# anonymousauthors001/SGS-GNN

Hardware: AMD Instinct MI355X
Metric: sampled edges/sec + training steps/sec, Reddit hybrid 20% sparsity (higher is better)
Workload: dtype f32

## Files before the change

include/sgs_hip.h:

```cpp
#ifndef SGS_HIP_H_
#define SGS_HIP_H_

#include <stddef.h>
#include <stdint.h>

#ifdef __cplusplus
extern "C" {
#endif

#define SGS_ABI_VERSION 1

#define SGS_OK 0
#define SGS_EINVAL (-1)
#define SGS_EWORKSPACE (-2)
#define SGS_EHIP (-3)

typedef void* sgs_stream_t;

int sgs_abi_version(void);
const char* sgs_last_error(void);

int sgs_rng_set_epoch_buffer(const uint64_t* epoch_dev);
int sgs_exp_noise(uint64_t seed, uint64_t stream_id, int64_t E, float* noise, sgs_stream_t stream);
int sgs_dropout_keep(uint64_t seed, uint32_t site, int64_t rows, int64_t cols, float p, uint8_t* keep,
// ... 74 lines not shown

int sgs_mean_weights(int64_t n_edges, int64_t N, const int32_t* in_ptr, const int32_t* out_ptr, const int32_t* out_dst,
                     float* what_in, float* what_out, sgs_stream_t stream);
int sgs_degree_prior_logits(const int64_t* edge_index, int64_t E, int64_t N, const int32_t* in_ptr,
                            const int32_t* out_ptr, float* logits, sgs_stream_t stream);

size_t sgs_gcn_norm_bwd_workspace_bytes(int64_t N);
int sgs_gcn_norm_bwd(const float* w, const float* gw_hat, const float* gloop, int64_t n_edges, int64_t N,
                     const float* dis, const float* loopw, const int32_t* in_ptr, const int32_t* in_src,
                     const int32_t* in_eid, const int32_t* out_ptr, const int32_t* out_dst, const int32_t* out_eid,
                     const int32_t* loop_eid, const int64_t* edge_index, float* dw, void* ws, size_t ws_bytes,
                     sgs_stream_t stream);
int sgs_gcn_norm_bwd_sum(const float* w, const float* gw_hat, const float* gloop, const float* gw_hat2, const float* gloop2, const float* dw_add,
                         int64_t n_edges, int64_t N, const float* dis, const float* loopw, const int32_t* in_ptr, const int32_t* in_src,
                         const int32_t* in_eid, const int32_t* out_ptr, const int32_t* out_dst, const int32_t* out_eid,
                         const int32_t* loop_eid, const int64_t* edge_index, float* dw, void* ws, size_t ws_bytes, sgs_stream_t stream);

int sgs_gcn_norm_bwd_node(const float* w, const float* gw_hat, const float* gloop, int64_t n_edges, int64_t N,
                          const float* dis, const float* loopw, const int32_t* in_ptr, const int32_t* in_src,
                          const int32_t* in_eid, const int32_t* out_ptr, const int32_t* out_dst, const int32_t* out_eid,
                          float* Hn, sgs_stream_t stream);
int sgs_gcn_norm_bwd_edge(const float* gw_hat, const float* gloop, int64_t n_edges, int64_t N, const float* dis,
                          const int32_t* loop_eid, const int64_t* edge_index, const float* Hn, float* dw,
                          sgs_stream_t stream);

#define SGS_ACT_NONE 0
#define SGS_ACT_RELU 1
#define SGS_ACT_RELU_DROPOUT 2
int sgs_spmm_csr(const float* X, int64_t N, int64_t D, int64_t nnz, const int32_t* ptr, const int32_t* col, const float* val,
                 const float* diag, const float* bias, int act, float p_drop, uint64_t seed, uint32_t site, float* Y,
                 sgs_stream_t stream);

int sgs_sddmm_csr(const float* A, const float* B, int64_t N, int64_t D, int64_t nnz, const int32_t* ptr, const int32_t* col,
                  const int32_t* eid, float* g, float* gdiag, sgs_stream_t stream);

int sgs_spmm_csr_variant(int64_t N, int64_t D, int64_t nnz, int aligned16);
int sgs_sddmm_csr_variant(int64_t N, int64_t D, int64_t nnz, int aligned16);

int sgs_act_bwd(const float* dY, const float* Y, int64_t n, int act, float p_drop, float* dZ, sgs_stream_t stream);
size_t sgs_colsum_workspace_bytes(int64_t N, int64_t D);
int sgs_colsum(const float* A, int64_t N, int64_t D, float* out, void* ws, size_t ws_bytes, sgs_stream_t stream);
int sgs_act_bwd_colsum(const float* dY, const float* Y, int64_t N, int64_t D, int act, float p_drop, float* dZ, float* colsum, void* ws,
                       size_t ws_bytes, sgs_stream_t stream);

int sgs_colsum_variant(int64_t N, int64_t D, int fused_act);

int sgs_gcn_pair_ok(int64_t N, int64_t nnz, int64_t D);
int sgs_spmm_csr_next(const float* X, int64_t N, int64_t D, int64_t nnz, const int32_t* ptr, const int32_t* col, const float* val,
                      const float* diag, const float* bias, int act, float p_drop, uint64_t seed, uint32_t site, const float* Wn, int64_t Dn,
                      float* Y, float* Z, sgs_stream_t stream);
int sgs_spmm_csr_bwd_prev(const float* dZ, int64_t N, int64_t D, int64_t nnz, const int32_t* ptr, const int32_t* col, const float* val,
                          const float* diag, const float* W, int64_t Dp, const float* Yp, int act, float p_drop, float* dX, float* dZp,
                          float* colsum, sgs_stream_t stream);

size_t sgs_edge_score_workspace_bytes(int64_t N, int64_t H, int64_t E);
int sgs_edge_score_hidden_supported(int64_t H);
int sgs_edge_score_get_variant(void);
int sgs_edge_score_get_bwd_variant(void);
void sgs_edge_score_set_bwd_variant(int variant);
int sgs_edge_score_bwd_tile(void);
void sgs_edge_score_set_variant(int variant);
int sgs_edge_score_fwd(const float* codes, const float* U, int64_t N, int64_t H, const int64_t* edge_index, int64_t E,
                       int64_t edge_id_offset, const float* W1, const float* b1, const float* w2, const float* b2,
                       float p_drop, uint64_t seed, uint32_t site, float* p_out, void* ws, size_t ws_bytes,
                       sgs_stream_t stream);
size_t sgs_edge_mates_workspace_bytes(int64_t n_edges);
int sgs_edge_mates(const int64_t* edge_index, int64_t n_edges, int64_t N, const int32_t* out_ptr, const int32_t* out_dst,
                   const int32_t* out_eid, int32_t* mate, void* ws, size_t ws_bytes, sgs_stream_t stream);
int sgs_edge_score_paired_supported(int64_t H);
int sgs_edge_score_fwd_paired(const float* codes, const float* U, int64_t N, int64_t H, const int64_t* edge_index, int64_t E,
                              int64_t edge_id_offset, const int32_t* canon, int64_t M, const int32_t* mate, const float* W1, const float* b1,
                              const float* w2, const float* b2, float p_drop, uint64_t seed, uint32_t site, float* p_out, void* ws,
                              size_t ws_bytes, sgs_stream_t stream);
int sgs_edge_score_bwd_core(const float* codes, const float* U, int64_t N, int64_t H, const int64_t* edge_index,
                            int64_t E, int64_t edge_id_offset, const int64_t* active_eid, int64_t n_active, const float* grad_p,
                            const float* W1, const float* b1, const float* w2, const float* b2, float p_drop,
                            uint64_t seed, uint32_t site, float* dv, float* hdz_part, float* dz, float* feat, void* ws,
                            size_t ws_bytes, sgs_stream_t stream);
int sgs_edge_score_bwd_dfeat_supported(int64_t H);
int sgs_edge_score_bwd_dfeat(const float* dv, int64_t n, int64_t H, const float* W1, float* dfeat, void* ws, size_t ws_bytes,
                             sgs_stream_t stream);

int sgs_edge_score_bwd_bits_supported(int64_t H);
int sgs_edge_score_fwd_mask(const float* codes, const float* U, int64_t N, int64_t H, const int64_t* edge_index, int64_t E,
                            int64_t edge_id_offset, const int32_t* canon, int64_t M, const int32_t* mate, const float* W1, const float* b1,
                            const float* w2, const float* b2, float p_drop, uint64_t seed, uint32_t site, float* p_out, uint32_t* maskbits,
                            void* ws, size_t ws_bytes, sgs_stream_t stream);
int sgs_edge_score_bwd_prep(const float* codes, int64_t N, int64_t H, const int64_t* edge_index, int64_t E, const int64_t* active_eid,
                            int64_t n_active, const float* grad_p, const float* p, const uint32_t* maskbits, float* dz, uint32_t* dvbits,
                            float* feat, sgs_stream_t stream);
int sgs_edge_score_dw2_from_parts(const float* W1, const float* T_raw, const float* U, const float* R_raw, const float* b1, const float* c_raw,
                                  int64_t N, int64_t H, float p_drop, float* dw2, sgs_stream_t stream);
int sgs_edge_score_probe_set(int stagger, int prio, uint32_t mode_mask);
int sgs_edge_score_probe_trace(unsigned long long* buf);
size_t sgs_edge_score_epd_workspace_bytes(int64_t H);
int sgs_edge_score_epd_fwd(const float* A, int64_t N, int64_t H, const int64_t* edge_index, int64_t E, int64_t edge_id_offset, const float* W1,
                           const float* b1, const float* w2, const float* b2, float p_hidden, uint64_t seed, uint32_t site, float p_ep,
                           uint64_t seed_x, uint32_t site_x, uint64_t seed_y, uint32_t site_y, float* p_out, void* ws, size_t ws_bytes,
                           sgs_stream_t stream);
int sgs_edge_score_epd_bwd_core(const float* A, int64_t N, int64_t H, const int64_t* edge_index, int64_t E, int64_t edge_id_offset,
                                const int64_t* active_eid, int64_t n_active, const float* grad_p, const float* W1, const float* b1, const float* w2,
                                const float* b2, float p_hidden, uint64_t seed, uint32_t site, float p_ep, uint64_t seed_x, uint32_t site_x,
                                uint64_t seed_y, uint32_t site_y, float* dv, float* hdz_part, float* dz, float* feat2, void* ws, size_t ws_bytes,
                                sgs_stream_t stream);
int sgs_edge_score_epd_reduce(const float* dfeat2, const float* A, int64_t N, int64_t H, const int32_t* in_ptr, const int32_t* in_src,
                              const int32_t* in_eid, const int32_t* out_ptr, const int32_t* out_dst, const int32_t* out_eid,
// ... 261 lines not shown
```

sgs-gnn_amd/csrc/gcn.hip:

```cpp
#include "sgs_common.h"

namespace sgs {
size_t graph_sort_workspace_bytes(int64_t n, int64_t N);
size_t graph_src_sorted_workspace_bytes(int64_t n, int64_t N);
int graph_build_src_sorted(const int64_t* ei, int64_t n, int64_t N, int32_t* in_ptr, int32_t* in_src, int32_t* in_eid, int32_t* out_ptr,
                           int32_t* out_dst, int32_t* out_eid, int32_t* loop_eid, int32_t* unsorted_flag, void* ws, size_t ws_bytes,
                           hipStream_t stream);
int graph_build_by_sort(const int64_t* ei, int64_t n, int64_t N, int32_t* in_ptr, int32_t* in_src, int32_t* in_eid, int32_t* out_ptr,
                        int32_t* out_dst, int32_t* out_eid, int32_t* loop_eid, void* ws, size_t ws_bytes, hipStream_t stream);
}

namespace sgs {
namespace {

constexpr int kT = 256;
constexpr int kMaxLdsRow = 8192;

__global__ void __launch_bounds__(kT) count_degrees(const int64_t* __restrict__ ei, int64_t n_edges, int* __restrict__ cnt_in,
                                                   int* __restrict__ cnt_out, int* __restrict__ loop_eid) {
    const int64_t e = static_cast<int64_t>(blockIdx.x) * kT + threadIdx.x;
    if (e >= n_edges) return;
    const int s = static_cast<int>(ei[e]), d = static_cast<int>(ei[n_edges + e]);
    atomicAdd(&cnt_in[d], 1);
    atomicAdd(&cnt_out[s], 1);
// ... 948 lines not shown
    norm_deg_body(w ? w + d * q : nullptr, N, in_ptr + d * (N + 1), in_src + d * q, in_eid + d * q, loop_eid + d * N, dis + d * N, loopw + d * N);
}
__global__ void __launch_bounds__(kT) multi_norm_weights(const float* __restrict__ w, int64_t q, int64_t N, const int* __restrict__ in_ptr,
                                                        const int* __restrict__ in_src, const int* __restrict__ in_eid, const float* __restrict__ dis,
                                                        const float* __restrict__ loopw, float* __restrict__ what_in, float* __restrict__ what_loop) {
    const int64_t d = blockIdx.y;
    norm_weights_body(N, w ? w + d * q : nullptr, N, q, in_ptr + d * (N + 1), in_src + d * q, in_eid + d * q, nullptr, nullptr, nullptr, dis + d * N,
                      loopw + d * N, what_in + d * q, nullptr, what_loop + d * N);
}
template <int VEC, int LPR>
__global__ void __launch_bounds__(kT) multi_spmm_csr(const float* __restrict__ X, int64_t xs, int64_t N, int64_t D, int64_t nnz,
                                                    const int* __restrict__ ptr, const int* __restrict__ col, const float* __restrict__ val,
                                                    const float* __restrict__ diag, const float* __restrict__ bias, int act, float* __restrict__ Y) {
    const int64_t d = blockIdx.y;
    spmm_csr_body<VEC, LPR>(X + d * xs, N, D, ptr + d * (N + 1), col + d * nnz, val + d * nnz, diag ? diag + d * N : nullptr, bias, act, 1.0f, 0u,
                            uint64_t(0), 0u, nullptr, Y + d * N * D);
}
template <int VEC, int NW>
__global__ void __launch_bounds__(64 * NW) multi_spmm_csr_rowblock(const float* __restrict__ X, int64_t xs, int64_t N, int64_t D, int64_t nnz,
                                                                 const int* __restrict__ ptr, const int* __restrict__ col,
                                                                 const float* __restrict__ val, const float* __restrict__ diag,
                                                                 const float* __restrict__ bias, int act, float* __restrict__ Y) {
    const int64_t d = blockIdx.y;
    spmm_csr_rowblock_body<VEC, NW>(X + d * xs, N, D, ptr + d * (N + 1), col + d * nnz, val + d * nnz, diag ? diag + d * N : nullptr, bias, act,
                                    1.0f, 0u, uint64_t(0), 0u, nullptr, Y + d * N * D);
}

enum { kPairCol = 0, kPairFwd = 1, kPairBwd = 2 };
constexpr int kPairMaxD = 512;
constexpr int kPairWlds = 12288;
constexpr int kPairWpre = kPairWlds / 1024;
template <class FY, class FW>
__device__ __forceinline__ float lib_gemm_dot(int K, FY y, FW w) {
    const int Kmain = K / 16 * 16;
    float z = 0.f;
    if (Kmain > 0) {
        float ya[8], wa[8];
#pragma unroll
        for (int u = 0; u < 8; ++u) { const int k = 2 * (u & 3) + (u >> 2); ya[u] = y(k); wa[u] = w(k); }
        for (int b = 0; b < Kmain; b += 8) {
            const int nb = b + 8 < Kmain ? b + 8 : b;
            float yn[8], wn[8];
#pragma unroll
            for (int u = 0; u < 8; ++u) { const int k = nb + 2 * (u & 3) + (u >> 2); yn[u] = y(k); wn[u] = w(k); }
#pragma unroll
            for (int u = 0; u < 8; ++u) z = fmaf(ya[u], wa[u], z);
#pragma unroll
            for (int u = 0; u < 8; ++u) { ya[u] = yn[u]; wa[u] = wn[u]; }
        }
    }
    for (int k = Kmain; k < K; ++k) z = fmaf(y(k), w(k), z);
    return z;
}
template <int VEC, int NW, int MODE>
__global__ void __launch_bounds__(1024) spmm_rowgroup_pair(const float* __restrict__ X, int64_t N, int64_t D, const int* __restrict__ ptr,
                                                           const int* __restrict__ col, const float* __restrict__ val,
                                                           const float* __restrict__ diag, const float* __restrict__ bias, int act,
                                                           float drop_scale, uint32_t drop_thresh, uint64_t seed, uint32_t site,
                                                           const uint64_t* __restrict__ epoch, float* __restrict__ Y,
                                                           const float* __restrict__ Wn, int64_t Dn, const float* __restrict__ Yp,
                                                           float* __restrict__ Zn, int ncs, float* __restrict__ colsum) {
    using V = typename VecT<VEC>::type;
    constexpr int RG = 16 / NW;
    __shared__ float part[RG][NW][64 * VEC];
    __shared__ __align__(16) float ys[RG * kPairMaxD];
    __shared__ float wl[MODE == kPairFwd ? kPairWlds : 1];
    if (MODE != kPairFwd && static_cast<int>(blockIdx.x) < ncs) {
        if (D % 4 == 0) colsum_small_v4_body<false>(X, nullptr, N, D, SGS_ACT_NONE, 1.f, nullptr, colsum, blockIdx.x);
        else            colsum_small_body<false>(X, nullptr, N, D, SGS_ACT_NONE, 1.f, nullptr, colsum, blockIdx.x);
        return;
    }
    seed = fold_epoch(seed, epoch);
    const int lane = threadIdx.x & 63, wave = (threadIdx.x >> 6) % NW, grp = threadIdx.x / (64 * NW);
    const int64_t row0 = static_cast<int64_t>(blockIdx.x - ncs) * RG;
    const int64_t i = row0 + grp;
    const bool live = i < N;
    int b = 0, e = 0;
    float dg = 0.f;
    uint32_t rkey = 0;
    const int yact = MODE == kPairBwd ? SGS_ACT_NONE : act;
    if (live) {
        b = ptr[i];
        e = ptr[i + 1];
        dg = diag ? diag[i] : 0.f;
        rkey = dropout_row_key(seed, site, static_cast<uint64_t>(i));
    }
    const bool wlds = MODE == kPairFwd && Dn * D <= kPairWlds;
    float wpre[MODE == kPairFwd ? kPairWpre : 1];
    if (MODE == kPairFwd && wlds) {
#pragma unroll
        for (int u = 0; u < kPairWpre; ++u) {
            const int64_t idx = threadIdx.x + 1024 * u;
            wpre[u] = idx < Dn * D ? Wn[idx] : 0.f;
        }
    }
    for (int64_t cbase = 0; cbase < D; cbase += 64 * VEC) {
        const int64_t c0 = cbase + static_cast<int64_t>(lane) * VEC;
        const bool in = c0 < D;
        float acc[VEC];
#pragma unroll
        for (int v = 0; v < VEC; ++v) acc[v] = 0.f;
        if (in) {
            int k = b + wave;
            for (; k + 7 * NW < e; k += 8 * NW) {
                int j[8]; float w[8]; V x[8];
#pragma unroll
                for (int u = 0; u < 8; ++u) { j[u] = col[k + NW * u]; w[u] = val[k + NW * u]; }
#pragma unroll
                for (int u = 0; u < 8; ++u) x[u] = *reinterpret_cast<const V*>(X + static_cast<int64_t>(j[u]) * D + c0);
#pragma unroll
                for (int u = 0; u < 8; ++u) {
                    float xv[VEC];
                    *reinterpret_cast<V*>(xv) = x[u];
#pragma unroll
                    for (int v = 0; v < VEC; ++v) acc[v] = fmaf(w[u], xv[v], acc[v]);
                }
            }
            for (; k < e; k += NW) {
                float xv[VEC];
                *reinterpret_cast<V*>(xv) = *reinterpret_cast<const V*>(X + static_cast<int64_t>(col[k]) * D + c0);
                const float w = val[k];
#pragma unroll
                for (int v = 0; v < VEC; ++v) acc[v] = fmaf(w, xv[v], acc[v]);
            }
        }
#pragma unroll
        for (int v = 0; v < VEC; ++v) part[grp][wave][lane * VEC + v] = acc[v];
        __syncthreads();
        const int t = threadIdx.x % (64 * NW);
        if (live && t < 64 * VEC && cbase + t < D) {
            const int64_t c = cbase + t;
            float y = 0.f;
#pragma unroll
            for (int g = 0; g < NW; g += 4) y += (part[grp][g][t] + part[grp][g + 1][t]) + (part[grp][g + 2][t] + part[grp][g + 3][t]);
            if (diag) y = fmaf(dg, X[i * D + c], y);
            if (bias) y += bias[c];
            if (yact != SGS_ACT_NONE) y = fmaxf(y, 0.f);
            if (yact == SGS_ACT_RELU_DROPOUT) y = dropout_keep_col(rkey, static_cast<uint32_t>(c), drop_thresh) ? y * drop_scale : 0.f;
            Y[i * D + c] = y;
            ys[grp * D + c] = y;
        }
        __syncthreads();
    }
    if (MODE == kPairFwd) {
        if (wlds) {
#pragma unroll
            for (int u = 0; u < kPairWpre; ++u) {
                const int64_t idx = threadIdx.x + 1024 * u;
                if (idx < Dn * D) {
                    const int64_t o = idx / D, k = idx - o * D;
                    wl[k * Dn + o] = wpre[u];
                }
            }
            __syncthreads();
        }
// ... 464 lines not shown
    switch (var / 1000000) {
        case 1:
            hipLaunchKernelGGL(colsum_small<false>, dim3(cdiv(D, 16)), dim3(1024), 0, stream, A, static_cast<const float*>(nullptr), N, D, SGS_ACT_NONE, 1.f,
                               static_cast<float*>(nullptr), out);
            break;
        case 2:
            hipLaunchKernelGGL(colsum_small_v4<false>, dim3(cdiv(D, 16)), dim3(1024), 0, stream, A, static_cast<const float*>(nullptr), N, D, SGS_ACT_NONE,
                               1.f, static_cast<float*>(nullptr), out);
            break;
        case 3:
            hipLaunchKernelGGL(vecsum_small, dim3(1), dim3(1024), 0, stream, A, N, out);
            break;
        default: {
            Carver cv(ws);
            const int rows = var / 100 % 1000;
            const int64_t nchunk = cdiv(N, rows);
            float* part = cv.take<float>(static_cast<size_t>(nchunk + 1) * D);
            if (nchunk > 0)
                hipLaunchKernelGGL(colsum_partial, dim3(cdiv(D, 64), nchunk), dim3(kT), 0, stream, A, N, D, rows, part);
            if (var % 100 == 16) hipLaunchKernelGGL(colsum_final<16>, dim3(cdiv(D, 64)), dim3(1024), 0, stream, part, nchunk, D, out);
            else                 hipLaunchKernelGGL(colsum_final<4>, dim3(cdiv(D, 64)), dim3(kT), 0, stream, part, nchunk, D, out);
        }
    }
    SGS_LAUNCH_OK();
    return SGS_OK;
}


int sgs_act_bwd_colsum(const float* dY, const float* Y, int64_t N, int64_t D, int act, float p_drop, float* dZ, float* colsum, void* ws,
                       size_t ws_bytes, sgs_stream_t stream_) {
    hipStream_t stream = static_cast<hipStream_t>(stream_);
    SGS_REQUIRE(N >= 0 && D >= 0 && p_drop >= 0.f && p_drop < 1.f, SGS_EINVAL, "sgs_act_bwd_colsum: bad arguments");
    if (D == 0) return SGS_OK;
    SGS_REQUIRE(colsum && (N == 0 || (dZ && dY && (act == SGS_ACT_NONE || Y))), SGS_EINVAL, "sgs_act_bwd_colsum: null pointer");
    switch (sgs_colsum_variant(N, D, 1) / 1000000) {
        case 1:
            hipLaunchKernelGGL(colsum_small<true>, dim3(cdiv(D, 16)), dim3(1024), 0, stream, dY, Y, N, D, act, 1.0f / (1.0f - p_drop), dZ, colsum);
            break;
        case 2:
            hipLaunchKernelGGL(colsum_small_v4<true>, dim3(cdiv(D, 16)), dim3(1024), 0, stream, dY, Y, N, D, act, 1.0f / (1.0f - p_drop), dZ, colsum);
            break;
        default:
            if (int rc = sgs_act_bwd(dY, Y, N * D, act, p_drop, dZ, stream_)) return rc;
            return sgs_colsum(dZ, N, D, colsum, ws, ws_bytes, stream_);
    }
    SGS_LAUNCH_OK();
    return SGS_OK;
}

int sgs_gcn_pair_ok(int64_t N, int64_t nnz, int64_t D) {
    return (N > 0 && N <= 65536 && nnz >= 16 * N && D > 0 && D <= kPairMaxD) ? 1 : 0;
}

#define PAIR_LAUNCH(MODE, grid, ...)                                                                                              \
    do {                                                                                                                          \
        if (vec == 4 && wide)  hipLaunchKernelGGL((spmm_rowgroup_pair<4, 16, MODE>), dim3(grid), dim3(1024), 0, stream, __VA_ARGS__); \
        else if (vec == 4)     hipLaunchKernelGGL((spmm_rowgroup_pair<4, 4, MODE>), dim3(grid), dim3(1024), 0, stream, __VA_ARGS__);  \
        else if (wide)         hipLaunchKernelGGL((spmm_rowgroup_pair<1, 16, MODE>), dim3(grid), dim3(1024), 0, stream, __VA_ARGS__); \
        else                   hipLaunchKernelGGL((spmm_rowgroup_pair<1, 4, MODE>), dim3(grid), dim3(1024), 0, stream, __VA_ARGS__);  \
    } while (0)

int sgs_spmm_csr_next(const float* X, int64_t N, int64_t D, int64_t nnz, const int32_t* ptr, const int32_t* col, const float* val,
                      const float* diag, const float* bias, int act, float p_drop, uint64_t seed, uint32_t site, const float* Wn, int64_t Dn,
                      float* Y, float* Z, sgs_stream_t stream_) {
    hipStream_t stream = static_cast<hipStream_t>(stream_);
    SGS_REQUIRE(sgs_gcn_pair_ok(N, nnz, D) && Dn > 0, SGS_EINVAL, "sgs_spmm_csr_next: not a row-block shape (see sgs_gcn_pair_ok)");
    SGS_REQUIRE(act >= SGS_ACT_NONE && act <= SGS_ACT_RELU_DROPOUT && p_drop >= 0.f && p_drop < 1.f, SGS_EINVAL,
                "sgs_spmm_csr_next: bad activation / dropout");
    SGS_REQUIRE(X && ptr && Y && Wn && Z && X != Y && Z != Y && Z != X, SGS_EINVAL, "sgs_spmm_csr_next: null or aliased pointer");
    const int vec = (D % 4 == 0 && aligned16(X) && aligned16(Y)) ? 4 : 1;
    const bool wide = nnz >= 256 * N;
    const float scale = 1.0f / (1.0f - p_drop);
    const uint32_t th = dropout_thresh(p_drop);
    if (act == SGS_ACT_RELU_DROPOUT && p_drop == 0.f) act = SGS_ACT_RELU;
    const int64_t grid = cdiv(N, wide ? 1 : 4);
    PAIR_LAUNCH(kPairFwd, grid, X, N, D, ptr, col, val, diag, bias, act, scale, th, seed, site, epoch_ptr(), Y, Wn, Dn,
                static_cast<const float*>(nullptr), Z, 0, static_cast<float*>(nullptr));
    SGS_LAUNCH_OK();
    return SGS_OK;
}

int sgs_spmm_csr_bwd_prev(const float* dZ, int64_t N, int64_t D, int64_t nnz, const int32_t* ptr, const int32_t* col, const float* val,
                          const float* diag, const float* W, int64_t Dp, const float* Yp, int act, float p_drop, float* dX, float* dZp,
                          float* colsum, sgs_stream_t stream_) {
    hipStream_t stream = static_cast<hipStream_t>(stream_);
    SGS_REQUIRE(sgs_gcn_pair_ok(N, nnz, D), SGS_EINVAL, "sgs_spmm_csr_bwd_prev: not a row-block shape (see sgs_gcn_pair_ok)");
    SGS_REQUIRE(act >= SGS_ACT_NONE && act <= SGS_ACT_RELU_DROPOUT && p_drop >= 0.f && p_drop < 1.f, SGS_EINVAL,
                "sgs_spmm_csr_bwd_prev: bad activation / dropout");
    SGS_REQUIRE(dZ && ptr && dX && dZ != dX, SGS_EINVAL, "sgs_spmm_csr_bwd_prev: null or aliased pointer");
    SGS_REQUIRE(!W || (Dp > 0 && dZp && (act == SGS_ACT_NONE || Yp) && dZp != dX && dZp != dZ), SGS_EINVAL,
                "sgs_spmm_csr_bwd_prev: W needs Dp > 0, dZp and (with an activation) Yp");
    const int vec = (D % 4 == 0 && aligned16(dZ) && aligned16(dX)) ? 4 : 1;
    const bool wide = nnz >= 256 * N;
    const int ncs = colsum ? static_cast<int>(cdiv(D, 16)) : 0;
    const int64_t grid = ncs + cdiv(N, wide ? 1 : 4);
    const float scale = 1.0f / (1.0f - p_drop);
    if (W)
        PAIR_LAUNCH(kPairBwd, grid, dZ, N, D, ptr, col, val, diag, static_cast<const float*>(nullptr), act, scale, 0u, uint64_t(0), 0u,
                    static_cast<const uint64_t*>(nullptr), dX, W, Dp, Yp, dZp, ncs, colsum);
    else
        PAIR_LAUNCH(kPairCol, grid, dZ, N, D, ptr, col, val, diag, static_cast<const float*>(nullptr), SGS_ACT_NONE, 1.f, 0u, uint64_t(0), 0u,
                    static_cast<const uint64_t*>(nullptr), dX, static_cast<const float*>(nullptr), int64_t(0), static_cast<const float*>(nullptr),
                    static_cast<float*>(nullptr), ncs, colsum);
    SGS_LAUNCH_OK();
    return SGS_OK;
}
#undef PAIR_LAUNCH

}

extern "C" {

size_t sgs_graph_filter_multi_workspace_bytes(int64_t E_parent, int64_t N, int64_t D) {
    if (E_parent < 0) E_parent = 0;
    if (N < 0) N = 0;
    if (D < 1) D = 1;
    return 2 * carve_bytes(static_cast<size_t>(D * (N + 1)), 4) + carve_bytes(static_cast<size_t>(D * E_parent + 1), 4) + 256;
}

int sgs_graph_filter_multi(const int32_t* pin_ptr, const int32_t* pin_src, const int32_t* pin_eid, int64_t E_parent, int64_t N, int64_t D,
                           const uint8_t* mask, const int64_t* sampled_eid, int64_t q, int32_t* in_ptr, int32_t* in_src, int32_t* in_eid,
                           int32_t* loop_eid, void* ws, size_t ws_bytes, sgs_stream_t stream_) {
    hipStream_t stream = static_cast<hipStream_t>(stream_);
    SGS_REQUIRE(E_parent >= 0 && N >= 0 && q >= 0 && q <= E_parent && E_parent < (int64_t(1) << 31) && N < (int64_t(1) << 30) && D >= 1 &&
                    D <= 65535, SGS_EINVAL, "sgs_graph_filter_multi: bad sizes");
    if (N == 0) return SGS_OK;
    SGS_REQUIRE(pin_ptr && in_ptr && loop_eid && (E_parent == 0 || (pin_src && pin_eid && mask)) &&
                    (q == 0 || (sampled_eid && in_src && in_eid)), SGS_EINVAL, "sgs_graph_filter_multi: null pointer");
    SGS_REQUIRE(ws && ws_bytes >= sgs_graph_filter_multi_workspace_bytes(E_parent, N, D), SGS_EWORKSPACE,
                "sgs_graph_filter_multi: workspace too small");
    Carver cv(ws);
    int* cnt = cv.take<int>(D * (N + 1));
    int* cur = cv.take<int>(D * (N + 1));
    int* pos = cv.take<int>(D * E_parent + 1);
    const unsigned Du = static_cast<unsigned>(D);
    const int64_t n_row_blocks = cdiv(N * 64, kT);
    const dim3 g1(static_cast<unsigned>(n_row_blocks + cdiv(q, kT)), Du), g3(static_cast<unsigned>(n_row_blocks), Du), blk(kT);
    hipLaunchKernelGGL(multi_filter_count, g1, blk, 0, stream, pin_ptr, pin_eid, N, E_parent, mask, sampled_eid, q, n_row_blocks, cnt, pos);
    if (N <= kSelfScanRows) {
        hipLaunchKernelGGL(multi_filter_fill<true>, g3, blk, 0, stream, pin_ptr, pin_src, pin_eid, N, E_parent, q, mask, pos, in_ptr, in_src, in_eid,
                           loop_eid, static_cast<const int*>(cnt));
    } else {
        hipLaunchKernelGGL(multi_scan_counts, dim3(1, Du), dim3(1024), 0, stream, cnt, N, in_ptr, cur);
        hipLaunchKernelGGL(multi_filter_fill<false>, g3, blk, 0, stream, pin_ptr, pin_src, pin_eid, N, E_parent, q, mask, pos, in_ptr, in_src, in_eid,
                           loop_eid, static_cast<const int*>(cnt));
    }
    SGS_LAUNCH_OK();
    return SGS_OK;
}

int sgs_gcn_norm_fwd_multi(const float* w, int64_t q, int64_t N, int64_t D, const int32_t* in_ptr, const int32_t* in_src, const int32_t* in_eid,
                           const int32_t* loop_eid, float* dis, float* loopw, float* what_in, float* what_loop, sgs_stream_t stream_) {
    hipStream_t stream = static_cast<hipStream_t>(stream_);
    SGS_REQUIRE(N >= 0 && q >= 0 && D >= 1 && D <= 65535, SGS_EINVAL, "sgs_gcn_norm_fwd_multi: bad sizes");
    if (N == 0) return SGS_OK;
    SGS_REQUIRE(in_ptr && loop_eid && dis && loopw && what_loop && (q == 0 || (in_src && in_eid && what_in)), SGS_EINVAL,
                "sgs_gcn_norm_fwd_multi: null pointer");
    const dim3 g(static_cast<unsigned>(cdiv(N * 64, kT)), static_cast<unsigned>(D));
    hipLaunchKernelGGL(multi_norm_deg, g, dim3(kT), 0, stream, w, q, N, in_ptr, in_src, in_eid, loop_eid, dis, loopw);
// ... 64 lines not shown
```

sgs-gnn_amd/ops.py:

```python
from __future__ import annotations

import ctypes
import os

import numpy as np
import torch

from . import _lib

SAMPLE_LEARNED, SAMPLE_PRIOR = 0, 1
ACT_NONE, ACT_RELU, ACT_RELU_DROPOUT = 0, 1, 2

_workspaces = {}
_retired_workspaces = []
_pin_workspaces = False


def _need_gpu(*tensors):
    for t in tensors:
        if t is not None and not t.is_cuda:
            raise RuntimeError("sgs_gnn_amd: the SGS hot path runs only on a HIP device (got a CPU tensor); "
                               "there is no CPU fallback")


# ... 1859 lines not shown
            dbias = _colsum(dZ)
        return dx, dW, (_handle_grad(nm, g) if g is not None else None), dbias, None, None, None, None, None, None


def gcn_layer(x, W, bias, nm: Norm, act=ACT_NONE, p=0.0, seed=0, site=0, xl=None):
    _need_gpu(x, W, bias)
    if x.dtype != torch.float32 or x.dim() != 2 or x.shape[0] != nm.graph.N:
        raise RuntimeError("gcn_layer: x must be float32 [N, F]")
    return _GCNLayer.apply(x, W, nm.handle, bias, nm, act, float(p), int(seed), int(site), xl)


def _pair_ok(gr, *widths):
    L = _lib.lib()
    return all(L.sgs_gcn_pair_ok(gr.N, gr.n_edges, int(w)) for w in widths)


class _GCN2(torch.autograd.Function):

    @staticmethod
    def forward(ctx, x, W1, b1, W2, b2, handle, nm, act, p, seed, site, xl1):
        L = _lib.lib()
        gr = nm.graph
        if xl1 is None:
            xl1 = _x_wt(x, W1)
        N, H = xl1.shape
        C = W2.shape[0]
        fused = _pair_ok(gr, H, C) and xl1.is_contiguous() and W2.is_contiguous() and W2.shape[1] == H
        if fused:
            h = torch.empty(N, H, dtype=torch.float32, device=xl1.device)
            xl2 = torch.empty(N, C, dtype=torch.float32, device=xl1.device)
            _lib.check(L.sgs_spmm_csr_next(_ptr(xl1, torch.float32), N, H, gr.n_edges, _ptr(gr.in_ptr), _ptr(gr.in_src), _ptr(nm.what_in),
                                           _ptr(nm.what_loop), _ptr(b1), act, float(p), seed, site, _ptr(W2, torch.float32), C, _ptr(h),
                                           _ptr(xl2), _stream()), "sgs_spmm_csr_next")
        else:
            h = _spmm(xl1, gr.in_ptr, gr.in_src, nm.what_in, nm.what_loop, b1, act, p, seed, site, N, H, gr.n_edges)
            xl2 = h @ W2.t()
        out = _spmm(xl2, gr.in_ptr, gr.in_src, nm.what_in, nm.what_loop, b2, ACT_NONE, 0.0, 0, 0, N, C, gr.n_edges)
        ctx.nm, ctx.act, ctx.p, ctx.fused = nm, act, p, fused
        ctx.has_b1, ctx.has_b2, ctx.has_handle = b1 is not None, b2 is not None, handle is not None
        ctx.save_for_backward(x, W1, xl1, h, W2, xl2)
        ctx.mark_non_differentiable(xl1)
        ctx.set_materialize_grads(False)
        return out, xl1

    @staticmethod
    def backward(ctx, dout, _dxl_unused):
        L = _lib.lib()
        nm, gr = ctx.nm, ctx.nm.graph
        x, W1, xl1, h, W2, xl2 = ctx.saved_tensors
        N, H = h.shape
        C = W2.shape[0]
        need_x, need_W1, need_b1, need_W2, need_b2, need_g = (ctx.needs_input_grad[i] for i in range(6))
        need_b1, need_b2, need_g = need_b1 and ctx.has_b1, need_b2 and ctx.has_b2, need_g and ctx.has_handle
        dx = dW1 = db1 = dW2 = db2 = g = None
        dZ2 = dout.contiguous()
        f32 = dict(dtype=torch.float32, device=dZ2.device)

        def sddmm(dZ, xl, D):
            gg = torch.empty(gr.n_edges + gr.N, **f32)
            _lib.check(L.sgs_sddmm_csr(_ptr(dZ), _ptr(xl), N, D, gr.n_edges, _ptr(gr.in_ptr), _ptr(gr.in_src), _ptr(gr.in_eid),
                                       gg[:gr.n_edges].data_ptr(), gg[gr.n_edges:].data_ptr(), _stream()), "sgs_sddmm_csr")
            return gg

        want_1 = need_x or need_W1 or need_b1 or need_g
        dxl2 = dZ1 = None
        if want_1 or need_W2:
            dxl2 = torch.empty(N, C, **f32)
            if ctx.fused:
                dZ1 = torch.empty(N, H, **f32) if want_1 else None
                db2 = torch.empty(C, **f32) if need_b2 else None
                _lib.check(L.sgs_spmm_csr_bwd_prev(_ptr(dZ2), N, C, gr.n_edges, _ptr(gr.out_ptr), _ptr(gr.out_dst), _ptr(nm.what_out),
                                                   _ptr(nm.what_loop), _ptr(W2 if want_1 else None, torch.float32), H, _ptr(h), ctx.act,
                                                   float(ctx.p), _ptr(dxl2), _ptr(dZ1), _ptr(db2), _stream()), "sgs_spmm_csr_bwd_prev")
            else:
                dxl2 = _spmm(dZ2, gr.out_ptr, gr.out_dst, nm.what_out, nm.what_loop, None, ACT_NONE, 0.0, 0, 0, N, C, gr.n_edges)
        if need_W2:
            dW2 = _dyt_x(dxl2, h, W2.shape, leaf=(ctx, 3))
        if want_1 and not ctx.fused:
            dZ1h = dxl2 @ W2
            if need_b1:
                dZ1, db1 = _act_bwd_colsum(dZ1h, h, ctx.act, ctx.p)
            else:
                dZ1 = torch.empty_like(dZ1h)
                _lib.check(L.sgs_act_bwd(_ptr(dZ1h), _ptr(h), dZ1h.numel(), ctx.act, float(ctx.p), _ptr(dZ1), _stream()), "sgs_act_bwd")
        g2 = sddmm(dZ2, xl2, C) if need_g else None
        if need_b2 and db2 is None:
            db2 = _colsum(dZ2)
        if need_x or need_W1 or (need_b1 and db1 is None and ctx.fused):
            if ctx.fused:
                dxl1 = torch.empty(N, H, **f32)
                db1 = torch.empty(H, **f32) if need_b1 else None
                _lib.check(L.sgs_spmm_csr_bwd_prev(_ptr(dZ1), N, H, gr.n_edges, _ptr(gr.out_ptr), _ptr(gr.out_dst), _ptr(nm.what_out),
                                                   _ptr(nm.what_loop), None, 0, None, ACT_NONE, 0.0, _ptr(dxl1), None, _ptr(db1), _stream()),
                           "sgs_spmm_csr_bwd_prev")
            else:
                dxl1 = _spmm(dZ1, gr.out_ptr, gr.out_dst, nm.what_out, nm.what_loop, None, ACT_NONE, 0.0, 0, 0, N, H, gr.n_edges)
            if need_W1:
                dW1 = _dyt_x(dxl1, x, W1.shape, leaf=(ctx, 1))
            if need_x:
                dx = dxl1 @ W1
        g1 = sddmm(dZ1, xl1, H) if need_g else None
        if need_b1 and db1 is None:
            db1 = _colsum(dZ1)
        if need_g:
            r2, r1 = _handle_grad(nm, g2), _handle_grad(nm, g1)
            g = r2 if r1 is None else (r1 if r2 is None else r2 + r1)
        return dx, dW1, db1, dW2, db2, g, None, None, None, None, None, None


def gcn2(x, W1, b1, W2, b2, nm: Norm, act=ACT_RELU, p=0.0, seed=0, site=0, xl1=None):
    _need_gpu(x, W1, b1, W2, b2)
    if x.dtype != torch.float32 or x.dim() != 2 or x.shape[0] != nm.graph.N:
        raise RuntimeError("gcn2: x must be float32 [N, F]")
    return _GCN2.apply(x, W1, b1, W2, b2, nm.handle, nm, act, float(p), int(seed), int(site), xl1)


class MultiSampleResult:
    __slots__ = ("mask", "eid", "edge_index", "stats", "w", "D", "E", "q")


def sample_topq_multi(mode: int, p, prior, c: float, q: int, edge_index, D: int, noise=None, seed: int = 0, stream_id0: int = 0,
                      want_edge_index: bool = True, want_w: bool = False) -> MultiSampleResult:
    L = _lib.lib()
    _need_gpu(p, prior, edge_index, noise)
    if p is None and edge_index is None:
        raise RuntimeError("sample_topq_multi: uniform weights (p=None) need edge_index for the number of candidates")
    E = p.numel() if p is not None else edge_index.shape[1]
    dev = p.device if p is not None else edge_index.device
    D = int(D)
    if noise is not None and (noise.dim() != 2 or tuple(noise.shape) != (D, E)):
        raise RuntimeError(f"sample_topq_multi: noise must be [D={D}, E={E}]")
    r = MultiSampleResult()
    r.D, r.E, r.q = D, E, q
    r.mask = torch.empty(max(D, 1), E, dtype=torch.bool, device=dev)
    r.eid = torch.empty(max(D, 1), q, dtype=torch.int64, device=dev)
    r.edge_index = torch.empty(max(D, 1), 2, q, dtype=torch.int64, device=dev) if (want_edge_index and edge_index is not None) else None
    r.stats = torch.empty(max(D, 1), 4, dtype=torch.float32, device=dev)
    r.w = torch.empty(max(D, 1), q, dtype=torch.float32, device=dev) if want_w else None
    ws = workspace(L.sgs_sample_topq_multi_workspace_bytes(E, max(D, 1)), dev)
    _lib.check(L.sgs_sample_topq_multi(mode, _ptr(p, torch.float32), _ptr(prior, torch.float32), float(c), _ptr(noise, torch.float32), seed,
                                       stream_id0, D, E, q, _ptr(edge_index, torch.int64), _ptr(r.mask), _ptr(r.eid), _ptr(r.edge_index),
                                       _ptr(r.stats), _ptr(r.w), ws.data_ptr(), ws.numel(), _stream()), "sgs_sample_topq_multi")
    return r


def graph_filter_multi(parent: Graph, smp: MultiSampleResult):
    L = _lib.lib()
    D, q, N = smp.D, smp.q, parent.N
    dev = parent.edge_index.device
    i32 = dict(dtype=torch.int32, device=dev)
    in_ptr = torch.empty(D, N + 1, **i32)
    in_src = torch.empty(D, max(q, 1), **i32)
    in_eid = torch.empty(D, max(q, 1), **i32)
    loop = torch.empty(D, max(N, 1), **i32)
# ... 440 lines not shown
```

Measured before the change: 103.5 million.

## Fuse SDDMM edge-gradient computation into backward row-group SpMM pair kernel

```diff
diff --git a/include/sgs_hip.h b/include/sgs_hip.h
--- a/include/sgs_hip.h
+++ b/include/sgs_hip.h
@@ -150,6 +150,10 @@
 int sgs_spmm_csr_bwd_prev(const float* dZ, int64_t N, int64_t D, int64_t nnz, const int32_t* ptr, const int32_t* col, const float* val,
                           const float* diag, const float* W, int64_t Dp, const float* Yp, int act, float p_drop, float* dX, float* dZp,
                           float* colsum, sgs_stream_t stream);
+int sgs_gcn_pair_sddmm_ok(int64_t N, int64_t nnz, int64_t D, int aligned16);
+int sgs_spmm_csr_bwd_prev_sddmm(const float* dZ, int64_t N, int64_t D, int64_t nnz, const int32_t* ptr, const int32_t* col, const int32_t* eid,
+                                const float* val, const float* diag, const float* W, int64_t Dp, const float* Yp, int act, float p_drop,
+                                const float* P, float* dX, float* dZp, float* colsum, float* g, float* gdiag, sgs_stream_t stream);
 
 size_t sgs_edge_score_workspace_bytes(int64_t N, int64_t H, int64_t E);
 int sgs_edge_score_hidden_supported(int64_t H);
diff --git a/sgs-gnn_amd/csrc/gcn.hip b/sgs-gnn_amd/csrc/gcn.hip
--- a/sgs-gnn_amd/csrc/gcn.hip
+++ b/sgs-gnn_amd/csrc/gcn.hip
@@ -1024,16 +1024,23 @@
     for (int k = Kmain; k < K; ++k) z = fmaf(y(k), w(k), z);
     return z;
 }
-template <int VEC, int NW, int MODE>
+struct PairSdd {
+    const float* P;
+    const int* eid;
+    float* g;
+    float* gdiag;
+};
+template <int VEC, int NW, int MODE, bool SDD = false>
 __global__ void __launch_bounds__(1024) spmm_rowgroup_pair(const float* __restrict__ X, int64_t N, int64_t D, const int* __restrict__ ptr,
                                                            const int* __restrict__ col, const float* __restrict__ val,
                                                            const float* __restrict__ diag, const float* __restrict__ bias, int act,
                                                            float drop_scale, uint32_t drop_thresh, uint64_t seed, uint32_t site,
                                                            const uint64_t* __restrict__ epoch, float* __restrict__ Y,
                                                            const float* __restrict__ Wn, int64_t Dn, const float* __restrict__ Yp,
-                                                           float* __restrict__ Zn, int ncs, float* __restrict__ colsum) {
+                                                           float* __restrict__ Zn, int ncs, float* __restrict__ colsum, PairSdd sdd) {
     using V = typename VecT<VEC>::type;
     constexpr int RG = 16 / NW;
+    static_assert(!SDD || MODE != kPairFwd, "the SDDMM side output belongs to the backward pairs");
     __shared__ float part[RG][NW][64 * VEC];
     __shared__ __align__(16) float ys[RG * kPairMaxD];
     __shared__ float wl[MODE == kPairFwd ? kPairWlds : 1];
@@ -1072,7 +1079,63 @@
         float acc[VEC];
 #pragma unroll
         for (int v = 0; v < VEC; ++v) acc[v] = 0.f;
-        if (in) {
+        if (SDD) {
+            const int64_t cl = in ? c0 : 0;
+            float a[VEC];
+#pragma unroll
+            for (int v = 0; v < VEC; ++v) a[v] = 0.f;
+            if (in && live) *reinterpret_cast<V*>(a) = *reinterpret_cast<const V*>(sdd.P + i * D + c0);
+            int k = b + wave;
+            for (; k + 7 * NW < e; k += 8 * NW) {
+                int j[8], ev[8]; float w[8]; V x[8];
+#pragma unroll
+                for (int u = 0; u < 8; ++u) { j[u] = col[k + NW * u]; w[u] = val[k + NW * u]; ev[u] = sdd.eid[k + NW * u]; }
+#pragma unroll
+                for (int u = 0; u < 8; ++u) x[u] = *reinterpret_cast<const V*>(X + static_cast<int64_t>(j[u]) * D + cl);
+                float d[8];
+#pragma unroll
+                for (int u = 0; u < 8; ++u) {
+                    float xv[VEC];
+                    *reinterpret_cast<V*>(xv) = x[u];
+                    float dd = 0.f;
+#pragma unroll
+                    for (int v = 0; v < VEC; ++v) {
+                        acc[v] = fmaf(w[u], xv[v], acc[v]);
+                        dd = fmaf(a[v], in ? xv[v] : 0.f, dd);
+                    }
+                    d[u] = dd;
+                }
+#pragma unroll
+                for (int u = 0; u < 8; ++u) d[u] = wave_sum_hi_dpp(d[u]);
+                if (lane == 63) {
+#pragma unroll
+                    for (int u = 0; u < 8; ++u) sdd.g[ev[u]] = d[u];
+                }
+            }
+            for (; k < e; k += NW) {
+                float xv[VEC];
+                *reinterpret_cast<V*>(xv) = *reinterpret_cast<const V*>(X + static_cast<int64_t>(col[k]) * D + cl);
+                const float w = val[k];
+                const int ev = sdd.eid[k];
+                float dd = 0.f;
+#pragma unroll
+                for (int v = 0; v < VEC; ++v) {
+                    acc[v] = fmaf(w, xv[v], acc[v]);
+                    dd = fmaf(a[v], in ? xv[v] : 0.f, dd);
+                }
+                dd = wave_sum_hi_dpp(dd);
+                if (lane == 63) sdd.g[ev] = dd;
+            }
+            if (wave == 0 && live && sdd.gdiag) {
+                float xv[VEC];
+                *reinterpret_cast<V*>(xv) = *reinterpret_cast<const V*>(X + i * D + cl);
+                float dd = 0.f;
+#pragma unroll
+                for (int v = 0; v < VEC; ++v) dd = fmaf(a[v], xv[v], dd);
+                dd = wave_sum_all(in ? dd : 0.f);
+                if (lane == 0) sdd.gdiag[i] = dd;
+            }
+        } else if (in) {
             int k = b + wave;
             for (; k + 7 * NW < e; k += 8 * NW) {
                 int j[8]; float w[8]; V x[8];
@@ -1643,13 +1706,14 @@
     return (N > 0 && N <= 65536 && nnz >= 16 * N && D > 0 && D <= kPairMaxD) ? 1 : 0;
 }
 
-#define PAIR_LAUNCH(MODE, grid, ...)                                                                                              \
-    do {                                                                                                                          \
-        if (vec == 4 && wide)  hipLaunchKernelGGL((spmm_rowgroup_pair<4, 16, MODE>), dim3(grid), dim3(1024), 0, stream, __VA_ARGS__); \
-        else if (vec == 4)     hipLaunchKernelGGL((spmm_rowgroup_pair<4, 4, MODE>), dim3(grid), dim3(1024), 0, stream, __VA_ARGS__);  \
-        else if (wide)         hipLaunchKernelGGL((spmm_rowgroup_pair<1, 16, MODE>), dim3(grid), dim3(1024), 0, stream, __VA_ARGS__); \
-        else                   hipLaunchKernelGGL((spmm_rowgroup_pair<1, 4, MODE>), dim3(grid), dim3(1024), 0, stream, __VA_ARGS__);  \
+#define PAIR_LAUNCH_SDD(MODE, SDD, grid, ...)                                                                                          \
+    do {                                                                                                                               \
+        if (vec == 4 && wide)  hipLaunchKernelGGL((spmm_rowgroup_pair<4, 16, MODE, SDD>), dim3(grid), dim3(1024), 0, stream, __VA_ARGS__); \
+        else if (vec == 4)     hipLaunchKernelGGL((spmm_rowgroup_pair<4, 4, MODE, SDD>), dim3(grid), dim3(1024), 0, stream, __VA_ARGS__);  \
+        else if (wide)         hipLaunchKernelGGL((spmm_rowgroup_pair<1, 16, MODE, SDD>), dim3(grid), dim3(1024), 0, stream, __VA_ARGS__); \
+        else                   hipLaunchKernelGGL((spmm_rowgroup_pair<1, 4, MODE, SDD>), dim3(grid), dim3(1024), 0, stream, __VA_ARGS__);  \
     } while (0)
+#define PAIR_LAUNCH(MODE, grid, ...) PAIR_LAUNCH_SDD(MODE, false, grid, __VA_ARGS__)
 
 int sgs_spmm_csr_next(const float* X, int64_t N, int64_t D, int64_t nnz, const int32_t* ptr, const int32_t* col, const float* val,
                       const float* diag, const float* bias, int act, float p_drop, uint64_t seed, uint32_t site, const float* Wn, int64_t Dn,
@@ -1666,36 +1730,62 @@
     if (act == SGS_ACT_RELU_DROPOUT && p_drop == 0.f) act = SGS_ACT_RELU;
     const int64_t grid = cdiv(N, wide ? 1 : 4);
     PAIR_LAUNCH(kPairFwd, grid, X, N, D, ptr, col, val, diag, bias, act, scale, th, seed, site, epoch_ptr(), Y, Wn, Dn,
-                static_cast<const float*>(nullptr), Z, 0, static_cast<float*>(nullptr));
-    SGS_LAUNCH_OK();
-    return SGS_OK;
-}
-
-int sgs_spmm_csr_bwd_prev(const float* dZ, int64_t N, int64_t D, int64_t nnz, const int32_t* ptr, const int32_t* col, const float* val,
-                          const float* diag, const float* W, int64_t Dp, const float* Yp, int act, float p_drop, float* dX, float* dZp,
-                          float* colsum, sgs_stream_t stream_) {
-    hipStream_t stream = static_cast<hipStream_t>(stream_);
-    SGS_REQUIRE(sgs_gcn_pair_ok(N, nnz, D), SGS_EINVAL, "sgs_spmm_csr_bwd_prev: not a row-block shape (see sgs_gcn_pair_ok)");
+                static_cast<const float*>(nullptr), Z, 0, static_cast<float*>(nullptr), PairSdd{});
+    SGS_LAUNCH_OK();
+    return SGS_OK;
+}
+
+static int spmm_csr_bwd_prev_impl(const char* who, const float* dZ, int64_t N, int64_t D, int64_t nnz, const int32_t* ptr, const int32_t* col,
+                                  const float* val, const float* diag, const float* W, int64_t Dp, const float* Yp, int act, float p_drop,
+                                  float* dX, float* dZp, float* colsum, const PairSdd* sdd, hipStream_t stream) {
+    SGS_REQUIRE(sgs_gcn_pair_ok(N, nnz, D), SGS_EINVAL, "%s: not a row-block shape (see sgs_gcn_pair_ok)", who);
     SGS_REQUIRE(act >= SGS_ACT_NONE && act <= SGS_ACT_RELU_DROPOUT && p_drop >= 0.f && p_drop < 1.f, SGS_EINVAL,
-                "sgs_spmm_csr_bwd_prev: bad activation / dropout");
-    SGS_REQUIRE(dZ && ptr && dX && dZ != dX, SGS_EINVAL, "sgs_spmm_csr_bwd_prev: null or aliased pointer");
+                "%s: bad activation / dropout", who);
+    SGS_REQUIRE(dZ && ptr && dX && dZ != dX, SGS_EINVAL, "%s: null or aliased pointer", who);
     SGS_REQUIRE(!W || (Dp > 0 && dZp && (act == SGS_ACT_NONE || Yp) && dZp != dX && dZp != dZ), SGS_EINVAL,
-                "sgs_spmm_csr_bwd_prev: W needs Dp > 0, dZp and (with an activation) Yp");
-    const int vec = (D % 4 == 0 && aligned16(dZ) && aligned16(dX)) ? 4 : 1;
+                "%s: W needs Dp > 0, dZp and (with an activation) Yp", who);
+    const int vec = (D % 4 == 0 && aligned16(dZ) && aligned16(dX) && (!sdd || aligned16(sdd->P))) ? 4 : 1;
     const bool wide = nnz >= 256 * N;
     const int ncs = colsum ? static_cast<int>(cdiv(D, 16)) : 0;
     const int64_t grid = ncs + cdiv(N, wide ? 1 : 4);
     const float scale = 1.0f / (1.0f - p_drop);
-    if (W)
-        PAIR_LAUNCH(kPairBwd, grid, dZ, N, D, ptr, col, val, diag, static_cast<const float*>(nullptr), act, scale, 0u, uint64_t(0), 0u,
-                    static_cast<const uint64_t*>(nullptr), dX, W, Dp, Yp, dZp, ncs, colsum);
-    else
-        PAIR_LAUNCH(kPairCol, grid, dZ, N, D, ptr, col, val, diag, static_cast<const float*>(nullptr), SGS_ACT_NONE, 1.f, 0u, uint64_t(0), 0u,
-                    static_cast<const uint64_t*>(nullptr), dX, static_cast<const float*>(nullptr), int64_t(0), static_cast<const float*>(nullptr),
-                    static_cast<float*>(nullptr), ncs, colsum);
-    SGS_LAUNCH_OK();
-    return SGS_OK;
-}
+    const float* const nof = nullptr;
+    const uint64_t* const noe = nullptr;
+    if (sdd) {
+        SGS_REQUIRE(D <= 64 * vec, SGS_EINVAL, "%s: a row must fit one pass of the wave (see sgs_gcn_pair_sddmm_ok)", who);
+        if (W) PAIR_LAUNCH_SDD(kPairBwd, true, grid, dZ, N, D, ptr, col, val, diag, nof, act, scale, 0u, uint64_t(0), 0u, noe, dX, W, Dp, Yp, dZp, ncs, colsum, *sdd);
+        else   PAIR_LAUNCH_SDD(kPairCol, true, grid, dZ, N, D, ptr, col, val, diag, nof, SGS_ACT_NONE, 1.f, 0u, uint64_t(0), 0u, noe, dX, nof, int64_t(0), nof,
+                               static_cast<float*>(nullptr), ncs, colsum, *sdd);
+    } else {
+        if (W) PAIR_LAUNCH(kPairBwd, grid, dZ, N, D, ptr, col, val, diag, nof, act, scale, 0u, uint64_t(0), 0u, noe, dX, W, Dp, Yp, dZp, ncs, colsum, PairSdd{});
+        else   PAIR_LAUNCH(kPairCol, grid, dZ, N, D, ptr, col, val, diag, nof, SGS_ACT_NONE, 1.f, 0u, uint64_t(0), 0u, noe, dX, nof, int64_t(0), nof,
+                           static_cast<float*>(nullptr), ncs, colsum, PairSdd{});
+    }
+    SGS_LAUNCH_OK();
+    return SGS_OK;
+}
+
+int sgs_spmm_csr_bwd_prev(const float* dZ, int64_t N, int64_t D, int64_t nnz, const int32_t* ptr, const int32_t* col, const float* val,
+                          const float* diag, const float* W, int64_t Dp, const float* Yp, int act, float p_drop, float* dX, float* dZp,
+                          float* colsum, sgs_stream_t stream_) {
+    return spmm_csr_bwd_prev_impl("sgs_spmm_csr_bwd_prev", dZ, N, D, nnz, ptr, col, val, diag, W, Dp, Yp, act, p_drop, dX, dZp, colsum, nullptr,
+                                  static_cast<hipStream_t>(stream_));
+}
+
+int sgs_gcn_pair_sddmm_ok(int64_t N, int64_t nnz, int64_t D, int al16) {
+    const int vec = (D % 4 == 0 && al16) ? 4 : 1;
+    return (sgs_gcn_pair_ok(N, nnz, D) && D <= 64 * vec) ? 1 : 0;
+}
+
+int sgs_spmm_csr_bwd_prev_sddmm(const float* dZ, int64_t N, int64_t D, int64_t nnz, const int32_t* ptr, const int32_t* col, const int32_t* eid,
+                                const float* val, const float* diag, const float* W, int64_t Dp, const float* Yp, int act, float p_drop,
+                                const float* P, float* dX, float* dZp, float* colsum, float* g, float* gdiag, sgs_stream_t stream_) {
+    SGS_REQUIRE(P && eid && g && col && val, SGS_EINVAL, "sgs_spmm_csr_bwd_prev_sddmm: null pointer");
+    const PairSdd sdd{P, eid, g, gdiag};
+    return spmm_csr_bwd_prev_impl("sgs_spmm_csr_bwd_prev_sddmm", dZ, N, D, nnz, ptr, col, val, diag, W, Dp, Yp, act, p_drop, dX, dZp, colsum, &sdd,
+                                  static_cast<hipStream_t>(stream_));
+}
+#undef PAIR_LAUNCH_SDD
 #undef PAIR_LAUNCH
 
 }
diff --git a/sgs-gnn_amd/ops.py b/sgs-gnn_amd/ops.py
--- a/sgs-gnn_amd/ops.py
+++ b/sgs-gnn_amd/ops.py
@@ -1935,7 +1935,7 @@
         C = W2.shape[0]
         need_x, need_W1, need_b1, need_W2, need_b2, need_g = (ctx.needs_input_grad[i] for i in range(6))
         need_b1, need_b2, need_g = need_b1 and ctx.has_b1, need_b2 and ctx.has_b2, need_g and ctx.has_handle
-        dx = dW1 = db1 = dW2 = db2 = g = None
+        dx = dW1 = db1 = dW2 = db2 = g = g1 = g2 = None
         dZ2 = dout.contiguous()
         f32 = dict(dtype=torch.float32, device=dZ2.device)
 
@@ -1944,6 +1944,20 @@
             _lib.check(L.sgs_sddmm_csr(_ptr(dZ), _ptr(xl), N, D, gr.n_edges, _ptr(gr.in_ptr), _ptr(gr.in_src), _ptr(gr.in_eid),
                                        gg[:gr.n_edges].data_ptr(), gg[gr.n_edges:].data_ptr(), _stream()), "sgs_sddmm_csr")
             return gg
+
+        def bwd_prev(dZ, D, W, Dp, Yp, act, p, xl, dX, dZp, colsum):
+            al16 = all(t.data_ptr() % 16 == 0 for t in (dZ, dX, xl))
+            if need_g and xl.is_contiguous() and L.sgs_gcn_pair_sddmm_ok(N, gr.n_edges, D, int(al16)):
+                gg = torch.empty(gr.n_edges + gr.N, **f32)
+                _lib.check(L.sgs_spmm_csr_bwd_prev_sddmm(_ptr(dZ), N, D, gr.n_edges, _ptr(gr.out_ptr), _ptr(gr.out_dst), _ptr(gr.out_eid),
+                                                         _ptr(nm.what_out), _ptr(nm.what_loop), _ptr(W, torch.float32), Dp, _ptr(Yp), act, p,
+                                                         _ptr(xl), _ptr(dX), _ptr(dZp), _ptr(colsum), gg[:gr.n_edges].data_ptr(),
+                                                         gg[gr.n_edges:].data_ptr(), _stream()), "sgs_spmm_csr_bwd_prev_sddmm")
+                return gg
+            _lib.check(L.sgs_spmm_csr_bwd_prev(_ptr(dZ), N, D, gr.n_edges, _ptr(gr.out_ptr), _ptr(gr.out_dst), _ptr(nm.what_out),
+                                               _ptr(nm.what_loop), _ptr(W, torch.float32), Dp, _ptr(Yp), act, p, _ptr(dX), _ptr(dZp),
+                                               _ptr(colsum), _stream()), "sgs_spmm_csr_bwd_prev")
+            return None
 
         want_1 = need_x or need_W1 or need_b1 or need_g
         dxl2 = dZ1 = None
@@ -1952,9 +1966,7 @@
             if ctx.fused:
                 dZ1 = torch.empty(N, H, **f32) if want_1 else None
                 db2 = torch.empty(C, **f32) if need_b2 else None
-                _lib.check(L.sgs_spmm_csr_bwd_prev(_ptr(dZ2), N, C, gr.n_edges, _ptr(gr.out_ptr), _ptr(gr.out_dst), _ptr(nm.what_out),
-                                                   _ptr(nm.what_loop), _ptr(W2 if want_1 else None, torch.float32), H, _ptr(h), ctx.act,
-                                                   float(ctx.p), _ptr(dxl2), _ptr(dZ1), _ptr(db2), _stream()), "sgs_spmm_csr_bwd_prev")
+                g2 = bwd_prev(dZ2, C, W2 if want_1 else None, H, h, ctx.act, float(ctx.p), xl2, dxl2, dZ1, db2)
             else:
                 dxl2 = _spmm(dZ2, gr.out_ptr, gr.out_dst, nm.what_out, nm.what_loop, None, ACT_NONE, 0.0, 0, 0, N, C, gr.n_edges)
         if need_W2:
@@ -1966,23 +1978,23 @@
             else:
                 dZ1 = torch.empty_like(dZ1h)
                 _lib.check(L.sgs_act_bwd(_ptr(dZ1h), _ptr(h), dZ1h.numel(), ctx.act, float(ctx.p), _ptr(dZ1), _stream()), "sgs_act_bwd")
-        g2 = sddmm(dZ2, xl2, C) if need_g else None
+        if need_g and g2 is None:
+            g2 = sddmm(dZ2, xl2, C)
         if need_b2 and db2 is None:
             db2 = _colsum(dZ2)
         if need_x or need_W1 or (need_b1 and db1 is None and ctx.fused):
             if ctx.fused:
                 dxl1 = torch.empty(N, H, **f32)
                 db1 = torch.empty(H, **f32) if need_b1 else None
-                _lib.check(L.sgs_spmm_csr_bwd_prev(_ptr(dZ1), N, H, gr.n_edges, _ptr(gr.out_ptr), _ptr(gr.out_dst), _ptr(nm.what_out),
-                                                   _ptr(nm.what_loop), None, 0, None, ACT_NONE, 0.0, _ptr(dxl1), None, _ptr(db1), _stream()),
-                           "sgs_spmm_csr_bwd_prev")
+                g1 = bwd_prev(dZ1, H, None, 0, None, ACT_NONE, 0.0, xl1, dxl1, None, db1)
             else:
                 dxl1 = _spmm(dZ1, gr.out_ptr, gr.out_dst, nm.what_out, nm.what_loop, None, ACT_NONE, 0.0, 0, 0, N, H, gr.n_edges)
             if need_W1:
                 dW1 = _dyt_x(dxl1, x, W1.shape, leaf=(ctx, 1))
             if need_x:
                 dx = dxl1 @ W1
-        g1 = sddmm(dZ1, xl1, H) if need_g else None
+        if need_g and g1 is None:
+            g1 = sddmm(dZ1, xl1, H)
         if need_b1 and db1 is None:
             db1 = _colsum(dZ1)
         if need_g:
```

New measurement: 105.1 million, median of 6. +1.5%, better.
